# torognes/vsearch

Measured on AMD Instinct MI355X. Metric: GCUPS (useful DP cells/s of the search16 global-alignment path: DP + traceback + CIGAR), higher is better.
Workload: dtype int16

## Files before the change

profiles/tb_stats.py:

```python
import argparse
import ctypes as C
import json
import os
import sys

import numpy as np
import torch

sys.path.insert(0, os.path.dirname(os.path.dirname(os.path.abspath(__file__))))
from vsearch_amd import Aligner, SequenceSet, _lib, workload

ap = argparse.ArgumentParser()
ap.add_argument("--queries", type=int, default=100_000)
ap.add_argument("--qlen", type=int, default=250)
ap.add_argument("--db", type=int, default=1_000_000)
ap.add_argument("--dlen", type=int, default=1000)
a = ap.parse_args()
dev = torch.device("cuda", 0)
db_ascii, db_off, db_len, fam = workload.make_family_db(a.db, a.dlen, seed=17, device=dev)
q_ascii, q_off, q_len, src = workload.make_queries(db_ascii, db_off, db_len, a.queries, a.qlen, seed=11, device=dev)
qidx, tidx = workload.family_candidates(src, fam, per_query=8, seed=5)
torch.cuda.synchronize()
lib = _lib.load()
lib.vsx_internal_tb_stats.argtypes = [C.POINTER(C.c_ulonglong), C.c_int]
out = (C.c_ulonglong * 16)()
with Aligner(device=0) as al:
    T = SequenceSet(al, blob=db_ascii.numel(), offsets=db_off, lengths=db_len, device_ptr=db_ascii.data_ptr())
    Q = SequenceSet(al, blob=q_ascii.numel(), offsets=q_off, lengths=q_len, device_ptr=q_ascii.data_ptr())
    plan = al.plan(Q, T, qidx, tidx)
    lib.vsx_internal_tb_stats(out, 1)
    plan.run()
    tm = plan.sync()
    lib.vsx_internal_tb_stats(out, 1)
    info = plan.describe()
    plan.close()
it, busy, distinct, walked, trips, pairs = (int(out[k]) for k in range(6))
print(json.dumps({"shape": [a.qlen, a.dlen], "pairs": pairs, "tasks": info["tasks"], "rows": info["rows_dominant"],
                  "wave_iterations": it, "busy_pair_tiles": busy, "tiles_per_pair": round(busy / max(pairs, 1), 2),
                  "iterations_per_wave": round(it / max(pairs / 64, 1), 2), "lane_utilisation": round(busy / max(it * 64, 1), 3),
                  "distinct_task_tiles": distinct, "pairs_per_distinct_tile": round(busy / max(distinct, 1), 2),
                  "cells_walked": walked, "cells_walked_per_pair_tile": round(walked / max(busy, 1), 2),
                  "traceback_ms_instrumented": round(tm.traceback_ms, 3),
                  "phase_cycles_per_wave_iteration(load1,recompute1,walk1,load2,recompute2,walk2)": [round(int(out[8 + k]) / max(it, 1)) for k in range(6)],
                  "kernel_cycles_per_wave": round(int(out[15]) / max(pairs / 64, 1))}))
```

vsearch_amd/csrc/vsx_device.hip:

```cpp
#include <hip/hip_runtime.h>
#include <type_traits>
#include <cstdlib>
#include <atomic>
#include "vsx_internal.h"

typedef unsigned int u32;
typedef unsigned int u32x4 __attribute__((ext_vector_type(4)));
typedef unsigned int u32x3 __attribute__((ext_vector_type(3)));
typedef short s2 __attribute__((ext_vector_type(2)));
typedef unsigned short us2 __attribute__((ext_vector_type(2)));

#define DEV __device__ __forceinline__
struct __attribute__((aligned(4))) Pair2 { unsigned int x, y; };

#define SIGN2 0x80008000u

DEV s2 S2(u32 x) { return __builtin_bit_cast(s2, x); }
DEV us2 U2(u32 x) { return __builtin_bit_cast(us2, x); }
DEV u32 UI(s2 x) { return __builtin_bit_cast(u32, x); }
DEV u32 UI(us2 x) { return __builtin_bit_cast(u32, x); }

DEV u32 sadd(u32 a, u32 b) { return UI(__builtin_elementwise_add_sat(S2(a), S2(b))); }
DEV u32 ssub(u32 a, u32 b) { return UI(__builtin_elementwise_sub_sat(S2(a), S2(b))); }
DEV u32 pmax(u32 a, u32 b) { return UI(__builtin_elementwise_max(S2(a), S2(b))); }
// ... 1041 lines not shown
              u32 cv = vin((u32) (uint16_t) P.hleft[ii < 0 ? 0 : ii]);
              if (TOPPAD && L == 0 && xs < pad) cv = vin((u32) (uint16_t) (((xs == pad - 1) ? 0 : -P.top_open) + (xs - pad - 1) * tl));
              tbL[64 + tid] = cv;
            }
        }
      else if (L == 0)
        {
#pragma unroll
          for (int cc = 0; cc < 17; ++cc)
            {
              int c = c0 - 1 + cc;
              if (c > jj) c = jj;
              const u32 corner = (u32) (uint16_t) (((TOPPAD && pad > 0) ? -P.top_open : 0) - (pad + 2) * tl);
              tbL[(cc + 1) * 64 + tid] = (c < 0) ? vin(corner) : vin((u32) (uint16_t) (P.htop[c] - pad * tl));
            }
        }
      else
        {
          const int Lp = L - 1;
          const int sp = Lp >> 4, lp = Lp & 15;
          stage_top(rowck + (size_t) VSX_CK_SLOT(CK8, g, lp) * (CK8 ? 3 : 4), VSX_ROWCK_PAIR_DW(CK8), (long) ((size_t) sp * steps) + (long) (c0 - 1 + lp),
                    (long) (rowsteps >> 1) - 1);
          if (c0 == 0) tbL[64 + tid] = vin((u32) (uint16_t) P.hleft[i0 - 1]);
        }
      stage_symbols(c0);

      u32 hp[RT], ee[RT], qa[RT];
      const u32 qrq_i = pen_pk(P.qrq_i_pk);
      const u32 rq_i = pen_pk(P.rq_i_pk);
      const bool lastrow_here = lastpos && (!MID || hh == 1);
      const u32 qrq_last = lastrow_here ? pen_pk(P.qrq_r_pk) : qrq_i;
      const u32 rq_last = lastrow_here ? pen_pk(P.rq_r_pk) : rq_i;
      if (m == 0)
        {
#pragma unroll
          for (int x = 0; x < RT; ++x)
            {
              int ii = i0 + r0h + x; if (ii > Q - 1) ii = Q - 1;
              if (ii < 0) ii = 0;
              const u32 hl = vin((u32) (uint16_t) P.hleft[ii]);
              hp[x] = hl;
              ee[x] = A::sub(hl, (ii < Q - 1) ? qrq_i : pen_pk(P.qrq_r_pk));
            }
          if (TOPPAD && L == 0 && pad > 0)
            {
#pragma unroll
              for (int x = 0; x < RT; ++x)
                if (r0h + x < pad)
                  {
                    const int xs = r0h + x;
                    const int sh = (xs - pad - 1) * tl;
                    hp[x] = vin((u32) (uint16_t) (((xs == pad - 1) ? 0 : -P.top_open) + sh));
                    ee[x] = A::sub(vin((u32) (uint16_t) (-P.top_open - P.top_step + sh)), qrq_i);
                  }
            }
        }
      else
        {
          if (CK8)
            {
              constexpr int NBQ = MID ? VSX_COLCK_NBH(RT) : VSX_COLCK_NB(R, true);
              Quad fq[NBQ];
              if (MID)
                {
                  const u32 * cb = colck + ((size_t) s * nblk + (size_t) (m - 1)) * COL_DW + VSX_COLCK_CDW(VSX_COLCK_NB(R, true), VSX_CK_SLOT(true, g, l), 0)
                                   + (size_t) (hh * NBQ) * (4 * VSX_COLCK_CG);
#pragma unroll
                  for (int b = 0; b < NBQ; ++b) fq[b] = *reinterpret_cast<const Quad *>(cb + (size_t) b * (4 * VSX_COLCK_CG));
                }
              else
                {
                  const u32 * cb = colck + ((size_t) s * nblk + (size_t) (m - 1)) * COL_DW + VSX_COLCK_CDW(VSX_COLCK_NB(R, true), VSX_CK_SLOT(true, g, l), 0);
#pragma unroll
                  for (int b = 0; b < NBQ; ++b) fq[b] = *reinterpret_cast<const Quad *>(cb + (size_t) b * (4 * VSX_COLCK_CG));
                }
              auto flat = [&](int z) -> u32 {
                const Quad & qd = fq[z >> 2];
                return (z & 3) == 0 ? qd.x : (z & 3) == 1 ? qd.y : (z & 3) == 2 ? qd.z : qd.w;
              };
#pragma unroll
              for (int x = 0; x < RT; ++x)
                {
                  const u32 h = half_lo(flat(x), hi) & 0xffffu;
                  const u32 dd = flat(RT + (x >> 1)) >> (8 * ((x & 1) * 2 + (hi ? 1 : 0)));
                  hp[x] = h;
                  ee[x] = h - (u32) (int) (int8_t) (dd & 0xffu);
                }
            }
          else if (R % 2 == 0)
            {
              const u32 * cb = colck + ((size_t) s * nblk + (size_t) (m - 1)) * COL_DW + VSX_COLCK_DW(R, g * 16 + l, 0);
              constexpr int NBQ = (2 * R) / 4 ? (2 * R) / 4 : 1;
              Quad fq[NBQ];
#pragma unroll
              for (int b = 0; b < NBQ; ++b) fq[b] = *reinterpret_cast<const Quad *>(cb + (size_t) b * (4 * VSX_COLCK_G));
              auto flat = [&](int z) -> u32 {
                const Quad & qd = fq[z >> 2];
                return (z & 3) == 0 ? qd.x : (z & 3) == 1 ? qd.y : (z & 3) == 2 ? qd.z : qd.w;
              };
#pragma unroll
              for (int x = 0; x < R; ++x) { hp[x] = inck(half_lo(flat(x), hi)); ee[x] = inck(half_lo(flat(R + x), hi)); }
            }
          else
            {
#pragma unroll
              for (int x = 0; x < R; ++x)
                {
                  hp[x] = inck(half_lo(colck_at(s, m - 1, g * 16 + l, x), hi));
                  ee[x] = inck(half_lo(colck_at(s, m - 1, g * 16 + l, R + x), hi));
                }
            }
        }
      {
        u32 w[(RT + 3) / 4];
#pragma unroll
        for (int e = 0; e < (RT + 3) / 4; ++e) w[e] = *reinterpret_cast<const u32_unaligned *>(q + i0 + r0h + 4 * e);
#pragma unroll
        for (int x = 0; x < RT; ++x)
          qa[x] = (w[x >> 2] >> (8 * (x & 3))) & 15u;
        if (TOPPAD && L == 0)
          {
#pragma unroll
            for (int x = 0; x < RT; ++x)
              if (r0h + x < pad) qa[x] = 16u;
          }
      }
      u32 diag = tbL[64 + tid] & 0xffffu;

      const bool tile_int = CK8 && RT > 1 && RT <= 16 && !__any(busy && (c0 + cmax >= D - 1));
      const bool top_is_border = (L == 0) && (hh == 0);
      for (int cc = 0; cc <= cmax; ++cc)
        {
          const int c = c0 + cc;
          const u32 qrt = (c < D - 1) ? qrt_i16 : qrt_r16;
          const u32 rt = (c < D - 1) ? rt_i16 : rt_r16;
          const u32 tbv = tbL[(cc + 2) * 64 + tid];
          const u32 topH = tbv & 0xffffu;
          u32 F = top_is_border ? A::sub(topH, qrt) : (tbv >> 16);
          const u32 b16 = (((u32) symL[(cc >> 1) * 64 + tid] >> (4 * (cc & 1))) & 15u) * 32u;
          u32 Hd = diag;
          u32 acc = 0;
          auto row = [&](int x, auto int_tag) __attribute__((always_inline)) {
            constexpr bool INT = decltype(int_tag)::value;
            const u32 V = A::score((int16_t) Ssh[b16 + qa[x]]);
            const u32 h0 = A::add(Hd, V);
            const u32 dU = A::dif(h0, F);
            const u32 h1 = A::max(h0, F);
            const u32 dL = A::dif(h1, ee[x]);
            const u32 h2 = A::max(h1, ee[x]);
            Hd = hp[x];
            hp[x] = h2;
            const bool plain = INT && x < RT - 1;
            const u32 qrq = (x == RT - 1) ? qrq_last : qrq_i;
            const u32 rq = (x == RT - 1) ? rq_last : rq_i;
            const u32 hf = A::sub(h2, qrt);
            const u32 f = INT ? F : A::sub(F, rt);
            const u32 dEU = A::dif(hf, f);
            F = A::max(f, hf);
            const u32 he = plain ? hf : A::sub(h2, qrq);
            const u32 e = plain ? ee[x] : A::sub(ee[x], rq);
            const u32 dEL = A::dif(he, e);
            ee[x] = A::max(e, he);
            acc = A::fun(A::fun(A::fun(A::fun(acc, dU), dL), dEU), dEL);
          };
          if (one_row)
            {
              row(0, std::false_type {});
              bitsL[(cc * ND) * 64 + tid] = (uint16_t) A::one_row_word(acc);
            }
          else
            {
#pragma unroll
              for (int x4 = 0; x4 < RT; x4 += 4)
                if (x4 <= rmax)
                  {
                    if (tile_int)
                      {
#pragma unroll
                        for (int y = 0; y < 4; ++y)
                          if (x4 + y < RT) row(x4 + y, std::true_type {});
                      }
                    else
                      {
#pragma unroll
                        for (int y = 0; y < 4; ++y)
                          if (x4 + y < RT) row(x4 + y, std::false_type {});
                      }
                    bitsL[(cc * ND + (x4 >> 2)) * 64 + tid] = (uint16_t) acc;
                  }
            }
          diag = topH;
        }

      if (busy)
        {
          while (r >= r0h && j >= c0 && (!TOPPAD || i >= 0))
            {
              const int cw = j - c0;
              const int rv = r - r0h;
              const u32 w = bitsL[(cw * ND + (rv >> 2)) * 64 + tid];
              int rid = RT - 4 * (rv >> 2);
              if (rid > 4) rid = 4;
              const u32 bts = A::nibble(w, rid, rv & 3);
              ++al;
              if (op == 1 && (bts & A::EXT_LEFT)) { --j; push(1); }
              else if (op == 2 && (bts & A::EXT_UP)) { --i; --r; push(2); }
              else if (bts & A::LEFT) { if (op != 1) ++ga; --j; push(1); }
              else if (bts & A::UP) { if (op != 2) ++ga; --i; --r; push(2); }
              else { --i; --r; --j; push(0); }
#if VSX_TB_STATS
              atomicAdd(&vsx_tb_stats_dev[3], 1ull);
#endif
            }
          if (r < 0 && L > 0) { --L; r = (L == 0 ? rtop0 : R) - 1; }
        }
    }
#if VSX_TB_STATS
  if (valid) atomicAdd(&vsx_tb_stats_dev[5], 1ull);
#endif
  if (!valid) return;

  VsxPairOut o;
  o.pad = 0; o.nruns = 0; o.run_off = 0;
  if (so.overflow)
    {
      o.score = 32767; o.aligned = 0; o.matches = 0; o.mismatches = 0; o.gaps = 0;
      out[pair_ids[k]] = o;
      rank_note(FL, pair_ids[k], 0u, 32767, 0.0);
      return;
    }
  if (i >= 0) { al += (u32) (i + 1); if (op != 2) ++ga; push_n(2, (u32) (i + 1)); }
  if (j >= 0) { al += (u32) (j + 1); if (op != 1) ++ga; push_n(1, (u32) (j + 1)); }
  if (op >= 0) my[nruns++] = (runlen << 2) | (u32) op;

  u32 ma = 0, mi = 0;
  {
    int qi = Q - 1, tj = D - 1;
    for (u32 x = 0; x < nruns; ++x)
      {
        const u32 w = my[x];
        const int len = (int) (w >> 2);
        const u32 o2 = w & 3u;
        if (o2 == 0)
          {
            for (int b = 0; b < len; b += 8)
              {
                const int rem = (len - b < 8) ? len - b : 8;
                const unsigned long long aw = *reinterpret_cast<const u64_unaligned *>(q + (qi - b - 7));
                const unsigned long long cw = *reinterpret_cast<const u64_unaligned *>(d + (tj - b - 7));
                const unsigned long long ones = 0x0101010101010101ull;
                const unsigned long long x = aw & cw;
                unsigned long long t = (x | (x >> 1) | (x >> 2) | (x >> 3)) & ones;
                if (P.n_mismatch)
                  {
                    const unsigned long long a15 = aw & (aw >> 1) & (aw >> 2) & (aw >> 3);
                    const unsigned long long c15 = cw & (cw >> 1) & (cw >> 2) & (cw >> 3);
                    t &= ~(a15 | c15);
                  }
                t &= ~0ull << (8 * (8 - rem));
                const u32 m8 = (u32) __builtin_popcountll(t);
                ma += m8;
                mi += (u32) rem - m8;
              }
            qi -= len; tj -= len;
          }
        else if (o2 == 1) tj -= len;
        else qi -= len;
      }
  }

  u32 verdict = 0;
  double idv = 0.0;
  if (FL.enabled && nruns > 0) verdict = accept_verdict(FL, Q, D, (int) al, (int) ma, (int) mi, (int) ga, my[nruns - 1], my[0], &idv);
  if (verdict == 3u) nruns = 0;
  rank_note(FL, pair_ids[k], verdict, (int) so.score, idv);

  const unsigned long long base = atomicAdd(cursor, (unsigned long long) nruns);
  if (base + nruns <= runs_capacity)
    for (u32 x = 0; x < nruns; ++x) runs[base + x] = my[x];

  o.score = so.score;
  o.aligned = (uint16_t) al; o.matches = (uint16_t) ma; o.mismatches = (uint16_t) mi; o.gaps = (uint16_t) ga;
  o.pad = (uint16_t) verdict;
  o.nruns = nruns;
  o.run_off = base;
  out[pair_ids[k]] = o;
}


DEV u32 pk_add(u32 a, u32 b) { return UI((us2) (U2(a) + U2(b))); }
DEV u32 pk_sub(u32 a, u32 b) { return psubw(a, b); }
#ifdef VSX_TB2_WAVES_N
#define VSX_TB2_WAVES(R_, MID_) VSX_TB2_WAVES_N
#endif
#ifndef VSX_TB2_WAVES
#define VSX_TB2_WAVES(R_, MID_) 3
#endif
#ifndef VSX_TB_LDSSTAGE
#define VSX_TB_LDSSTAGE 1
#endif
#ifndef VSX_TB_LDSSTAGE_FOR
#define VSX_TB_LDSSTAGE_FOR(R_) ((R_) == 14 || (R_) == 16 || (R_) >= 26)
#endif
template <int R, bool MID>
__global__ void __launch_bounds__(64) __attribute__((amdgpu_waves_per_eu(VSX_TB2_WAVES(R, MID), 8)))
vsx_traceback_tilt_kernel(const VsxDevParams P, const VsxFilterDev FL, const VsxTask * __restrict__ tasks,
                          const u32 * __restrict__ pair_slot, const u32 * __restrict__ pair_ids, u32 npairs,
                          const uint8_t * __restrict__ qc, const uint8_t * __restrict__ tc,
                          const u32 * __restrict__ ck, const VsxSlotOut * __restrict__ slot,
                          u32 * __restrict__ slab, const uint64_t * __restrict__ slab_off,
                          u32 * __restrict__ runs, uint64_t runs_capacity, unsigned long long * cursor,
                          VsxPairOut * __restrict__ out)
{
  static_assert(R >= 4 && (!MID || R % 2 == 0), "R = 1 keeps the first kernel");
  constexpr int RT = MID ? R / 2 : R;
  constexpr int HR = (RT + 1) / 2;
  constexpr int NG = (HR + 3) / 4;
  constexpr int XL = RT - 1 - HR;
  constexpr int NBQ = MID ? VSX_COLCK_NBH(RT) : VSX_COLCK_NB(R, true);
  __shared__ uint8_t Ssh[512];
  __shared__ u32 Ssh4[16];
  constexpr int BITS_DW = 17 * NG * 64, SYM_DW = 10 * 64 / 4;
  __shared__ __attribute__((aligned(16))) u32 arenaL[BITS_DW + SYM_DW + 19 * 64];
  u32 * const bitsL = arenaL;
  uint8_t * const symL = reinterpret_cast<uint8_t *>(arenaL + BITS_DW);
  u32 * const tbL = arenaL + BITS_DW + SYM_DW;
  constexpr bool LSTAGE = (VSX_TB_LDSSTAGE != 0) && VSX_TB_LDSSTAGE_FOR(R) && (BITS_DW + SYM_DW >= 9 * 64 * 4);
  const int tid = (int) threadIdx.x;
  for (int x = tid; x < 512; x += 64)
    Ssh[x] = (uint8_t) (((x & 31) < 16) ? P.matrix[(x >> 5) * 16 + (x & 15)] : (int16_t) (-P.top_step + 2 * P.tilt));
  if (tid < 16)
    {
      const int16_t * mr = P.matrix + tid * 16;
      Ssh4[tid] = (u32) (uint8_t) mr[1] | ((u32) (uint8_t) mr[2] << 8) | ((u32) (uint8_t) mr[4] << 16) | ((u32) (uint8_t) mr[8] << 24);
    }
  __syncthreads();

  const u32 k = blockIdx.x * 64 + (u32) threadIdx.x;
  const bool valid = k < npairs;
  const u32 ts = pair_slot[valid ? k : 0];
  const u32 task = ts >> 3, sl = ts & 7;
  const VsxTask & T = tasks[task];
  const VsxSlotOut so = slot[ts];
  const bool live = valid && !so.overflow;

  const int Q = (int) T.qlen;
  const int D = (int) T.tlen[sl];
  const u32 steps32 = T.steps;
  const unsigned long long dir_off = T.dir_off;
  constexpr size_t COL_DW = (size_t) 64 * 4 * VSX_COLCK_NB(R, true);
  const int g = (int) (sl >> 1) + (int) T.group0;
  const bool hi = (sl & 1) != 0;
  const u32 half_sel = hi ? 0x07060302u : 0x05040100u;
  const u32 bias = P.max3 ? 0x3E00u : 0x8000u;
  const u32 bias_pk = bias * 0x10001u;
  const int tl = P.tilt;
  auto pk16 = [](int v) -> u32 { const u32 x = (u32) v & 0xffffu; return x | (x << 16); };
  auto pk2 = [](int lo, int hi_) -> u32 { return ((u32) lo & 0xffffu) | ((u32) hi_ << 16); };
  const int qrt_i = P.qrt_i, qrt_r = P.qrt_r, rt_i = P.rt_i, rt_r = P.rt_r;
  const int qrq_i = (int) (int16_t) (P.qrq_i_pk & 0xffffu), rq_i = (int) (int16_t) (P.rq_i_pk & 0xffffu);
  const int qrq_r = (int) (int16_t) (P.qrq_r_pk & 0xffffu), rq_r = (int) (int16_t) (P.rq_r_pk & 0xffffu);
  const uint8_t * __restrict__ q = qc + T.qoff;
  const uint8_t * __restrict__ d = tc + T.toff[sl];
  u32 * __restrict__ my = slab + slab_off[valid ? k : 0];

  int i = live ? Q - 1 : -1, j = live ? D - 1 : -1;
  int L = (Q + R - 1) / R - 1;
  int r = R - 1;
  int op = -1;
  u32 runlen = 0, nruns = 0;
  u32 al = 0, ga = 0;
  auto push_n = [&](int newop, u32 n) {
    if (newop == op) { runlen += n; return; }
    if (op >= 0) my[nruns++] = (runlen << 2) | (u32) op;
    op = newop;
    runlen = n;
  };
  auto push = [&](int newop) { push_n(newop, 1u); };

  if (live)
    {
      const int lv = (so.leave == 0xFFFFu) ? -1 : (int) so.leave;
      if (lv < D - 1)
        {
          const u32 n = (u32) (D - 1 - lv);
          al += n; ++ga;
          push_n(1, n);
          j = lv;
        }
    }

  const u32 mA[4] = {0x01010101u, 0x02020202u, 0x04040404u, 0x08080808u};
  const u32 mB[4] = {0x10101010u, 0x20202020u, 0x40404040u, 0x80808080u};

#if VSX_TB_STATS
  const unsigned long long t_kernel0 = __builtin_readcyclecounter();
  unsigned n_iter = 0;
  unsigned long long tphase[6] = {0, 0, 0, 0, 0, 0};
#endif
  for (;;)
    {
      const bool busy = (i >= 0) && (j >= 0);
      if (!__any(busy)) break;
#if VSX_TB_STATS
      ++n_iter;
#endif

      u32 Qb = (u32) Q, stb = steps32;
      unsigned long long dob = dir_off;
      asm volatile("" : "+v"(Qb), "+v"(stb), "+v"(dob));
      const int total_lanes = ((int) Qb + R - 1) / R;
      const int rcnt0 = (int) Qb - (total_lanes - 1) * R;
      const int pad = R - rcnt0;
      const int nstrips = (total_lanes + 15) >> 4;
      const size_t steps = stb;
      const size_t nblk = (steps + 15) >> 4;
      const size_t rowsteps = ((size_t) nstrips * steps + 1) & ~(size_t) 1;
      const size_t rowck_dw = (rowsteps >> 1) * VSX_ROWCK_PAIR_DW(true);
      const u32 * __restrict__ rowck = ck + dob;
      const u32 * __restrict__ colck = rowck + rowck_dw;
      const u32 * __restrict__ midck = colck + (size_t) nstrips * nblk * COL_DW;
      const int s = L >> 4, l = L & 15;
      const int jj = busy ? j : 0;
      const int m = (jj + l) >> 4;
      const int c0 = (16 * m - l) > 0 ? 16 * m - l : 0;
      const int c0b = (m >= 1 && 16 * (m - 1) - l > 0) ? 16 * (m - 1) - l : 0;
      const int i0 = (L == 0) ? -pad : rcnt0 + (L - 1) * R;
      const bool lastpos = (L == total_lanes - 1);
      const int hh = (MID && busy && r >= RT) ? 1 : 0;
      const int r0h = hh * RT;
      const bool lastrow_here = lastpos && (!MID || hh == 1);
      const bool top_is_border = (L == 0) && (hh == 0);
#if VSX_TB_STATS & 1
      {
        const unsigned key = busy ? (((unsigned) task & 0x3FFu) << 22) | ((unsigned) L << 12) | ((unsigned) m << 1) | (unsigned) hh : 0xFFFFFFFFu;
        bool leader = busy;
        for (int o = 1; o < 8; ++o)
          {
            const unsigned other = (unsigned) __shfl((int) key, (tid & ~7) | ((tid - o) & 7), 64);
            if ((tid & 7) >= o && other == key) leader = false;
          }
        const unsigned long long nb = __popcll(__ballot(busy)), nl = __popcll(__ballot(leader));
        if (tid == 0) { atomicAdd(&vsx_tb_stats_dev[1], nb); atomicAdd(&vsx_tb_stats_dev[2], nl); }
      }
#endif

      struct TileIn { Trio v3[LSTAGE ? 1 : 9]; int par; Quad fq[NBQ]; u32 sw[5]; };
      auto load_tile = [&](TileIn & in, const int cst, const int mleft) __attribute__((always_inline)) {
        in.par = 0;
        if (!top_is_border)
          {
            const u32 * base;
            long gstart;
            if (MID && hh == 1)
              {
                base = midck + (size_t) VSX_CK_SLOT(true, g, l) * 3;
                gstart = (long) ((size_t) s * steps) + (long) (cst - 1 + l);
              }
            else
              {
                const int Lp = L - 1, sp = Lp >> 4, lp = Lp & 15;
                base = rowck + (size_t) VSX_CK_SLOT(true, g, lp) * 3;
                gstart = (long) ((size_t) sp * steps) + (long) (cst - 1 + lp);
              }
            const long p0 = gstart >> 1;
            in.par = (int) (gstart - 2 * p0);
            const u32 * bp = base + p0 * (long) VSX_ROWCK_PAIR_DW(true);
            if (LSTAGE)
              {
#pragma unroll
                for (int e = 0; e < 9; ++e)
                  __builtin_amdgcn_global_load_lds((const __attribute__((address_space(1))) void *) (bp + e * VSX_ROWCK_PAIR_DW(true)),
                                                   (__attribute__((address_space(3))) void *) (arenaL + e * 256), 12, 0, 0);
              }
            else
              {
#pragma unroll
            for (int e = 0; e < 9; ++e) in.v3[LSTAGE ? 0 : e] = *reinterpret_cast<const Trio *>(bp + e * VSX_ROWCK_PAIR_DW(true));
              }
          }
        const u32 * cb = colck + ((size_t) s * nblk + (size_t) (mleft > 0 ? mleft : 0)) * COL_DW + VSX_COLCK_CDW(VSX_COLCK_NB(R, true), VSX_CK_SLOT(true, g, l), 0)
                         + (MID ? (size_t) (hh * NBQ) * (4 * VSX_COLCK_CG) : 0);
#pragma unroll
        for (int b = 0; b < NBQ; ++b) in.fq[b] = *reinterpret_cast<const Quad *>(cb + (size_t) b * (4 * VSX_COLCK_CG));
#pragma unroll
        for (int e = 0; e < 5; ++e) in.sw[e] = *reinterpret_cast<const u32_unaligned *>(d + cst + 4 * e);
      };

      u32 qcd[HR], qsel[HR];
      bool plain_acgt = true;
      {
        u32 w[(RT + 3) / 4];
#pragma unroll
        for (int e = 0; e < (RT + 3) / 4; ++e) w[e] = *reinterpret_cast<const u32_unaligned *>(q + i0 + r0h + 4 * e);
        auto code_of = [&](int x) -> u32 {
          const int xx = x < RT ? x : RT - 1;
          u32 c = (w[xx >> 2] >> (8 * (xx & 3))) & 15u;
          if (L == 0 && r0h + xx < pad) c = 16u;
          return c;
        };
#pragma unroll
        for (int x = 0; x < HR; ++x)
          {
            const u32 a = code_of(x), b = code_of(x + HR);
            qcd[x] = a | (b << 16);
            const u32 ia = (a >> 1) - (a >> 3), ib = (b >> 1) - (b >> 3);
            qsel[x] = ia | 0x0C000C00u | ((4u + ib) << 16);
            plain_acgt = plain_acgt && (a == 1 || a == 2 || a == 4 || a == 8) && (b == 1 || b == 2 || b == 4 || b == 8);
          }
      }
      const bool fastV = !__any(busy && !plain_acgt);

      const u32 qrq_pk_i = pk16(qrq_i), rq_pk_i = pk16(rq_i);
      const u32 qrq_pk_x = pk2(qrq_i, lastrow_here ? qrq_r : qrq_i), rq_pk_x = pk2(rq_i, lastrow_here ? rq_r : rq_i);

      auto recompute = [&](const TileIn & in, const bool border_left, const int cst, const int rmax_raw, const int cmax, const bool tile_int)
                       __attribute__((always_inline)) {
        if (top_is_border)
          {
            const u32 corner = (u32) (uint16_t) (((pad > 0) ? -P.top_open : 0) - (pad + 2) * tl);
#pragma unroll
            for (int e = 0; e < 17; ++e)
              {
                int c = cst - 1 + e;
                if (c > jj) c = jj;
                tbL[e * 64 + tid] = (c < 0) ? (corner & 0xffffu) : (u32) (uint16_t) (P.htop[c] - pad * tl);
              }
          }
        else
          {
            u32 * dst = tbL + tid - in.par * 64;
            if (LSTAGE) asm volatile("s_waitcnt vmcnt(0)" ::: "memory");
#pragma unroll
            for (int e = 0; e < 9; ++e)
              {
                Trio raw;
                if (LSTAGE) raw = *reinterpret_cast<const Trio *>(arenaL + e * 256 + tid * 4);
                else raw = in.v3[LSTAGE ? 0 : e];
                const u32 h0 = (half_lo(raw.x, hi) - bias) & 0xffffu, h1 = (half_lo(raw.y, hi) - bias) & 0xffffu;
                const u32 dd = hi ? (raw.z >> 8) : raw.z;
                const int d0 = (int) (int8_t) (dd & 0xffu), d1 = (int) (int8_t) ((dd >> 16) & 0xffu);
                if (e > 0 || in.par == 0) dst[(2 * e) * 64] = h0 | ((h0 - (u32) d0) << 16);
                dst[(2 * e + 1) * 64] = h1 | ((h1 - (u32) d1) << 16);
              }
            if (cst == 0)
              {
                u32 cv;
                if (MID && hh == 1)
                  {
                    const int xs = RT - 1;
                    int ii = i0 + xs; if (ii > Q - 1) ii = Q - 1;
                    cv = (u32) (uint16_t) P.hleft[ii < 0 ? 0 : ii];
                    if (L == 0 && xs < pad) cv = (u32) (uint16_t) (((xs == pad - 1) ? 0 : -P.top_open) + (xs - pad - 1) * tl);
                  }
                else cv = (u32) (uint16_t) P.hleft[i0 - 1];
                tbL[tid] = cv;
              }
          }
#pragma unroll
        for (int c2 = 0; c2 < 10; ++c2)
          {
            const u32 lo = (in.sw[c2 >> 1] >> (16 * (c2 & 1))) & 15u, hi4 = (in.sw[c2 >> 1] >> (16 * (c2 & 1) + 8)) & 15u;
            symL[c2 * 64 + tid] = (uint8_t) (lo | (hi4 << 4));
          }
        u32 hp[HR], ee[HR];
        if (border_left)
          {
#pragma unroll
            for (int x = 0; x < HR; ++x)
              {
                u32 hv[2], ev[2];
#pragma unroll
                for (int hf_ = 0; hf_ < 2; ++hf_)
                  {
                    const int xs = r0h + x + hf_ * HR;
                    int ii = i0 + xs; if (ii > Q - 1) ii = Q - 1;
                    if (ii < 0) ii = 0;
                    asm volatile("" : "+v"(ii));
                    int hl = P.hleft[ii];
                    int e0 = hl - ((ii < Q - 1) ? qrq_i : qrq_r);
                    if (L == 0 && xs < pad)
                      {
                        const int sh = (xs - pad - 1) * tl;
                        hl = ((xs == pad - 1) ? 0 : -P.top_open) + sh;
                        e0 = -P.top_open - P.top_step + sh - qrq_i;
                      }
                    hv[hf_] = (u32) hl & 0xffffu; ev[hf_] = (u32) e0 & 0xffffu;
                  }
                hp[x] = hv[0] | (hv[1] << 16);
                ee[x] = ev[0] | (ev[1] << 16);
              }
          }
        else
          {
            auto flat = [&](int z) -> u32 {
              const Quad & qd = in.fq[z >> 2];
              return (z & 3) == 0 ? qd.x : (z & 3) == 1 ? qd.y : (z & 3) == 2 ? qd.z : qd.w;
            };
#pragma unroll
            for (int x = 0; x < HR; ++x)
              {
                const int xa = x, xb = (x + HR < RT) ? x + HR : RT - 1;
                const u32 h = pk_sub(__builtin_amdgcn_perm(flat(xb), flat(xa), half_sel), bias_pk);
                const int da = (int) (int8_t) ((flat(RT + (xa >> 1)) >> (8 * ((xa & 1) * 2 + (hi ? 1 : 0)))) & 0xffu);
                const int db = (int) (int8_t) ((flat(RT + (xb >> 1)) >> (8 * ((xb & 1) * 2 + (hi ? 1 : 0)))) & 0xffu);
                hp[x] = h;
                ee[x] = pk_sub(h, ((u32) da & 0xffffu) | ((u32) db << 16));
              }
          }
        const int xmax = rmax_raw >= HR ? HR - 1 : rmax_raw;
        u32 tb_prev = tbL[tid];
        u32 Hd_end = 0, F_end = 0;
        u32 cr_prev = 0, qrt_prev = 0, rt_prev = 0;
        auto sym_at = [&](int it) -> u32 { return ((u32) symL[(it >> 1) * 64 + tid] >> (4 * (it & 1))) & 15u; };
        const bool FASTV_any = fastV;
        u32 tbv_n = tbL[64 + tid];
        u32 cr_n = FASTV_any ? Ssh4[sym_at(0)] : sym_at(0) * 32u;
        u32 sy_n = sym_at(1);
        auto column = [&](const int it, auto int_tag, auto fast_tag, auto first_tag) __attribute__((always_inline)) {
          constexpr bool INT = decltype(int_tag)::value;
          constexpr bool FASTV = decltype(fast_tag)::value;
          constexpr bool FIRST = decltype(first_tag)::value;
          const int c = cst + it;
          const u32 tbv = tbv_n;
          const u32 cr = cr_n;
          cr_n = FASTV ? Ssh4[sy_n] : sy_n * 32u;
          tbv_n = tbL[(it + 2) * 64 + tid];
          sy_n = sym_at(it + 2);
          u32 qrt_pk = 0, rt_pk = 0;
          if (!INT)
            {
              const u32 ql = (u32) ((c < D - 1) ? qrt_i : qrt_r) & 0xffffu, rl = (u32) ((c < D - 1) ? rt_i : rt_r) & 0xffffu;
              qrt_pk = ql | (qrt_prev << 16); rt_pk = rl | (rt_prev << 16);
              qrt_prev = ql; rt_prev = rl;
            }
          else qrt_pk = pk16(qrt_i);
          u32 Hd = __builtin_amdgcn_perm(Hd_end, tb_prev, 0x05040100u);
          u32 F = __builtin_amdgcn_perm(F_end, tbv, 0x05040302u);
          if (top_is_border)
            F = __builtin_amdgcn_perm(F_end, ((tbv & 0xffffu) - (INT ? (u32) qrt_i : (qrt_pk & 0xffffu))), 0x05040100u);
#pragma unroll
          for (int g4 = 0; g4 < NG; ++g4)
            if (4 * g4 <= xmax)
              {
                u32 acc = 0;
#pragma unroll
                for (int x = 4 * g4; x < 4 * g4 + 4; ++x)
                  if (x < HR)
                    {
                      u32 V;
                      if (FASTV) V = __builtin_amdgcn_perm(cr_prev, cr, qsel[x]);
                      else
                        {
                          u32 qc2 = qcd[x];
                          asm volatile("" : "+v"(qc2));
                          V = (u32) Ssh[cr + (qc2 & 0xffffu)] | ((u32) Ssh[cr_prev + (qc2 >> 16)] << 16);
                        }
                      const u32 h0 = pk_add(Hd, V);
                      const u32 dU = ssub(h0, F);
                      const u32 h1 = pmax(h0, F);
                      const u32 dL = ssub(h1, ee[x]);
                      const u32 h2 = pmax(h1, ee[x]);
                      Hd = hp[x];
                      hp[x] = FIRST ? bfi(0x0000FFFFu, h2, hp[x]) : h2;
                      const u32 hf = pk_sub(h2, qrt_pk);
                      const u32 f = INT ? F : pk_sub(F, rt_pk);
                      const u32 dEU = ssub(hf, f);
                      F = pmax(f, hf);
                      const bool plain = INT && x != XL;
                      const u32 he = plain ? hf : pk_sub(h2, x == XL ? qrq_pk_x : qrq_pk_i);
                      const u32 e = plain ? ee[x] : pk_sub(ee[x], x == XL ? rq_pk_x : rq_pk_i);
                      const u32 dEL = ssub(he, e);
                      const u32 en = pmax(e, he);
                      ee[x] = FIRST ? bfi(0x0000FFFFu, en, ee[x]) : en;
                      acc = a_bfi(mA[x & 3], __builtin_amdgcn_perm(dL, dU, 0x0B0A0908u), acc);
                      acc = a_bfi(mB[x & 3], __builtin_amdgcn_perm(dEL, dEU, 0x0B0A0908u), acc);
                    }
                bitsL[(it * NG + g4) * 64 + tid] = acc;
              }
          Hd_end = Hd;
          F_end = F;
          tb_prev = tbv;
          cr_prev = cr;
        };
        auto sweep = [&](auto int_tag, auto fast_tag) __attribute__((always_inline)) {
          column(0, int_tag, fast_tag, std::true_type {});
          for (int it = 1; it <= cmax + 1; ++it) column(it, int_tag, fast_tag, std::false_type {});
        };
        if (tile_int) { if (fastV) sweep(std::true_type {}, std::true_type {}); else sweep(std::true_type {}, std::false_type {}); }
        else          { if (fastV) sweep(std::false_type {}, std::true_type {}); else sweep(std::false_type {}, std::false_type {}); }
      };
      auto walk = [&](const int cst) __attribute__((always_inline)) {
        while (r >= r0h && j >= cst && i >= 0)
          {
            const int cw = j - cst;
            const int rv = r - r0h;
            const bool up_half = rv >= HR;
            const int rx = up_half ? rv - HR : rv;
            const u32 w = bitsL[((cw + (up_half ? 1 : 0)) * NG + (rx >> 2)) * 64 + tid] >> ((rx & 3) + (up_half ? 8 : 0));
            ++al;
            const u32 inI = (op == 1) ? 1u : 0u, inD = (op == 2) ? 1u : 0u;
            const u32 c1 = inI & (w >> 20);
            const u32 c2 = (c1 ^ 1u) & inD & (w >> 4);
            const u32 c12 = c1 | c2;
            const u32 c3 = (c12 ^ 1u) & (w >> 16);
            const u32 c4 = ((c12 | c3) ^ 1u) & w;
            const u32 isI = (c1 | c3) & 1u, isD = (c2 | c4) & 1u;
            const int newop = (int) (isI + 2u * isD);
            ga += ((c3 & (inI ^ 1u)) | (c4 & (inD ^ 1u))) & 1u;
            j -= (int) (isD ^ 1u);
            const int di = (int) (isI ^ 1u);
            i -= di; r -= di;
            if (newop != op)
              {
                if (op >= 0) my[nruns++] = (runlen << 2) | (u32) op;
                op = newop;
                runlen = 0;
              }
            ++runlen;
#if VSX_TB_STATS & 1
            atomicAdd(&vsx_tb_stats_dev[3], 1ull);
#endif
          }
      };

#if VSX_TB_STATS & 2
#define TBMARK(k_) do { __builtin_amdgcn_s_waitcnt(0); const unsigned long long now_ = __builtin_readcyclecounter(); tphase[k_] += now_ - tmark; tmark = now_; } while (0)
      unsigned long long tmark = __builtin_readcyclecounter();
#else
#define TBMARK(k_) do { } while (0)
#endif
#pragma unroll 1
      for (int tno = 0; tno < 2; ++tno)
        {
          const bool need = (tno == 0) ? busy : (busy && (m >= 1) && (r >= r0h) && (i >= 0) && (j >= 0) && (j < c0));
          if (tno == 1 && !__any(need)) break;
          const int cst = tno ? c0b : c0;
          TileIn in;
          load_tile(in, cst, tno ? m - 2 : m - 1);
          TBMARK(3 * tno);
          const int rmax_raw = __builtin_amdgcn_readfirstlane(wave_max_i32(need ? r - r0h : 0));
          const int cmax = __builtin_amdgcn_readfirstlane(wave_max_i32(need ? j - cst : 0));
          const bool tile_int = tno ? true : !__any(busy && (c0 + cmax >= D - 1));
          recompute(in, tno ? (m <= 1) : (m == 0), cst, rmax_raw, cmax, tile_int);
          TBMARK(3 * tno + 1);
          if (need) walk(cst);
          TBMARK(3 * tno + 2);
        }
      if (busy && r < 0 && L > 0) { --L; r = R - 1; }
    }
#if VSX_TB_STATS
  if (valid) atomicAdd(&vsx_tb_stats_dev[5], 1ull);
  if (tid == 0)
    {
      atomicAdd(&vsx_tb_stats_dev[15], __builtin_readcyclecounter() - t_kernel0); atomicAdd(&vsx_tb_stats_dev[0], (unsigned long long) n_iter);
      for (int k2 = 0; k2 < 6; ++k2) atomicAdd(&vsx_tb_stats_dev[8 + k2], tphase[k2]);
    }
#endif
  if (!valid) return;

  VsxPairOut o;
  o.pad = 0; o.nruns = 0; o.run_off = 0;
  if (so.overflow)
    {
      o.score = 32767; o.aligned = 0; o.matches = 0; o.mismatches = 0; o.gaps = 0;
      out[pair_ids[k]] = o;
      rank_note(FL, pair_ids[k], 0u, 32767, 0.0);
      return;
    }
  if (i >= 0) { al += (u32) (i + 1); if (op != 2) ++ga; push_n(2, (u32) (i + 1)); }
  if (j >= 0) { al += (u32) (j + 1); if (op != 1) ++ga; push_n(1, (u32) (j + 1)); }
  if (op >= 0) my[nruns++] = (runlen << 2) | (u32) op;

  u32 ma = 0, mi = 0;
  {
    int qi = Q - 1, tj = D - 1;
    for (u32 x = 0; x < nruns; ++x)
      {
        const u32 w = my[x];
        const int len = (int) (w >> 2);
        const u32 o2 = w & 3u;
        if (o2 == 0)
          {
            for (int b = 0; b < len; b += 8)
              {
                const int rem = (len - b < 8) ? len - b : 8;
                const unsigned long long aw = *reinterpret_cast<const u64_unaligned *>(q + (qi - b - 7));
                const unsigned long long cw = *reinterpret_cast<const u64_unaligned *>(d + (tj - b - 7));
                const unsigned long long ones = 0x0101010101010101ull;
                const unsigned long long x2 = aw & cw;
                unsigned long long t = (x2 | (x2 >> 1) | (x2 >> 2) | (x2 >> 3)) & ones;
                if (P.n_mismatch)
                  {
                    const unsigned long long a15 = aw & (aw >> 1) & (aw >> 2) & (aw >> 3);
                    const unsigned long long c15 = cw & (cw >> 1) & (cw >> 2) & (cw >> 3);
                    t &= ~(a15 | c15);
                  }
                t &= ~0ull << (8 * (8 - rem));
                const u32 m8 = (u32) __builtin_popcountll(t);
                ma += m8;
                mi += (u32) rem - m8;
              }
            qi -= len; tj -= len;
          }
        else if (o2 == 1) tj -= len;
        else qi -= len;
      }
  }

  u32 verdict = 0;
  double idv = 0.0;
  if (FL.enabled && nruns > 0) verdict = accept_verdict(FL, Q, D, (int) al, (int) ma, (int) mi, (int) ga, my[nruns - 1], my[0], &idv);
  if (verdict == 3u) nruns = 0;
  rank_note(FL, pair_ids[k], verdict, (int) so.score, idv);

  const unsigned long long base = atomicAdd(cursor, (unsigned long long) nruns);
  if (base + nruns <= runs_capacity)
    for (u32 x = 0; x < nruns; ++x) runs[base + x] = my[x];

  o.score = so.score;
  o.aligned = (uint16_t) al; o.matches = (uint16_t) ma; o.mismatches = (uint16_t) mi; o.gaps = (uint16_t) ga;
  o.pad = (uint16_t) verdict;
  o.nruns = nruns;
  o.run_off = base;
  out[pair_ids[k]] = o;
}

DEV u32 map4(u32 ch)
{
  const u32 c = ch | 0x20u;
  if (((ch | 0x20u) < 'a') || ((ch | 0x20u) > 'z') || ((ch & 0xC0u) != 0x40u)) return 0;
  switch (c)
    {
    case 'a': return 1;  case 'b': return 14; case 'c': return 2;  case 'd': return 13;
    case 'g': return 4;  case 'h': return 11; case 'k': return 12; case 'm': return 3;
    case 'n': return 15; case 'r': return 5;  case 's': return 6;  case 't': return 8;
    case 'u': return 8;  case 'v': return 7;  case 'w': return 9;  case 'y': return 10;
    default: return 0;
    }
}

__global__ void __launch_bounds__(256)
vsx_encode_kernel(const uint8_t * __restrict__ ascii, uint8_t * __restrict__ codes, uint64_t nbytes)
{
  __shared__ uint8_t lut[256];
  lut[threadIdx.x] = (uint8_t) map4(threadIdx.x);
  __syncthreads();
  const uint64_t nvec = nbytes >> 4;
  const uint64_t stride = (uint64_t) gridDim.x * blockDim.x;
  for (uint64_t v = (uint64_t) blockIdx.x * blockDim.x + threadIdx.x; v < nvec; v += stride)
    {
      const uint4 in = reinterpret_cast<const uint4 *>(ascii)[v];
      u32 w[4] = {in.x, in.y, in.z, in.w};
      u32 o[4];
#pragma unroll
      for (int x = 0; x < 4; ++x)
        o[x] = (u32) lut[w[x] & 0xff] | ((u32) lut[(w[x] >> 8) & 0xff] << 8) |
               ((u32) lut[(w[x] >> 16) & 0xff] << 16) | ((u32) lut[w[x] >> 24] << 24);
      reinterpret_cast<uint4 *>(codes)[v] = make_uint4(o[0], o[1], o[2], o[3]);
    }
  if (blockIdx.x == 0 && threadIdx.x < (nbytes & 15))
    {
      const uint64_t p = (nvec << 4) + threadIdx.x;
      codes[p] = lut[ascii[p]];
    }
}

__global__ void __launch_bounds__(256)
vsx_purity_kernel(const uint8_t * __restrict__ codes, const uint64_t * __restrict__ off,
                  const uint32_t * __restrict__ len, uint64_t nseq, uint8_t * __restrict__ impure)
{
  const uint64_t s = (uint64_t) blockIdx.x * 4 + (threadIdx.x >> 6);
  if (s >= nseq) return;
  const int lane = threadIdx.x & 63;
  const uint8_t * p = codes + off[s];
  const uint32_t n = len[s];
  int bad = 0;
  for (uint32_t x = lane; x < n; x += 64)
    {
      const u32 c = p[x];
      bad |= !((c != 0) && ((c & (c - 1)) == 0));
    }
  const unsigned long long any = __ballot(bad);
  if (lane == 0) impure[s] = any ? 1 : 0;
}

__global__ void __launch_bounds__(256)
vsx_max3_selftest_kernel(u32 * bad)
{
  const u32 x = blockIdx.x * 256u + threadIdx.x;
  if (x > 0x7BFFu) return;
  const u32 edge[8] = {0u, 1u, 0x03FFu, 0x0400u, 0x3C00u, 0x3E00u, 0x7BFEu, 0x7BFFu};
  u32 wrong = 0;
  for (u32 k = 0; k < 64; ++k)
    {
      const u32 h = (x * 2654435761u) ^ (k * 0x9E3779B9u);
      const u32 y = (k < 8) ? edge[k] : (h >> 7) % 0x7C00u;
      const u32 z = (k < 16) ? edge[(k + 3) & 7] : (h >> 17) % 0x7C00u;
      const u32 a = x | (y << 16), b = y | (z << 16), c = z | (x << 16);
      const u32 got = pk_max3_bits(a, b, c);
      const u32 m = x > y ? (x > z ? x : z) : (y > z ? y : z);
      if (got != (m | (m << 16))) ++wrong;
      const u32 pa = h ^ (x << 13), pb = (h * 0x85EBCA6Bu) ^ k;
      const u32 pg = __builtin_amdgcn_perm(pa, pb, 0x0B0A0908u);
      const u32 pe = ((pb >> 15) & 1u) * 0xFFu | (((pb >> 31) & 1u) * 0xFFu) << 8 | (((pa >> 15) & 1u) * 0xFFu) << 16 | (((pa >> 31) & 1u) * 0xFFu) << 24;
      if (pg != pe) atomicAdd(bad + 1, 1u);
    }
  if (wrong) atomicAdd(bad, wrong);
}
static std::atomic<int> g_tb_v1_dev[65];
extern "C" void vsx_internal_set_tb_v2(int device, int on) { g_tb_v1_dev[device < 0 || device > 64 ? 64 : device].store(on ? 0 : 1); }
extern "C" hipError_t vsx_launch_max3_selftest(u32 * d_bad, hipStream_t st)
{
  hipLaunchKernelGGL(vsx_max3_selftest_kernel, dim3((0x7C00 + 255) / 256), dim3(256), 0, st, d_bad);
  return hipGetLastError();
}

static const int kRows[] = {1, 4, 8, 10, 12, 14, 16, 18, 20, 22, 24, 26, 28, 32};

extern "C" const int * vsx_supported_rows(int * count)
{
  *count = (int) (sizeof(kRows) / sizeof(kRows[0]));
  return kRows;
}

extern "C" hipError_t vsx_launch_encode(const uint8_t * d_ascii, uint8_t * d_codes, uint64_t nbytes, hipStream_t st)
{
  if (nbytes == 0) return hipSuccess;
  uint64_t blocks = ((nbytes >> 4) + 255) / 256;
  if (blocks < 1) blocks = 1;
  if (blocks > 256 * 8) blocks = 256 * 8;
  hipLaunchKernelGGL(vsx_encode_kernel, dim3((unsigned) blocks), dim3(256), 0, st, d_ascii, d_codes, nbytes);
  return hipGetLastError();
}

extern "C" hipError_t vsx_launch_purity(const uint8_t * d_codes, const uint64_t * d_off, const uint32_t * d_len,
                                        uint64_t nseq, uint8_t * d_impure, hipStream_t st)
{
  if (nseq == 0) return hipSuccess;
  hipLaunchKernelGGL(vsx_purity_kernel, dim3((unsigned) ((nseq + 3) / 4)), dim3(256), 0, st,
                     d_codes, d_off, d_len, nseq, d_impure);
  return hipGetLastError();
}

#define VSX_FWD_GO(GRID_, ...) hipLaunchKernelGGL((vsx_forward_kernel<__VA_ARGS__>), dim3(GRID_), dim3(64), 0, st, P, d_tasks, q, t, dir, strip, slot, ntasks)
#define VSX_FWD_GO4(GRID_, ...) hipLaunchKernelGGL((vsx_forward_kernel<__VA_ARGS__>), dim3(GRID_), dim3(256), 0, st, P, d_tasks, q, t, dir, strip, slot, ntasks)
template <int R>
static hipError_t launch_fwd2(int track, int nq, int one, const VsxDevParams & P, const VsxTask * d_tasks, uint32_t ntasks,
                              const uint8_t * q, const uint8_t * t, uint32_t * dir, uint2 * strip,
                              VsxSlotOut * slot, hipStream_t st)
{
  if (nq == 8)
    {
      if (!(P.tilt != 0 && !track) || (ntasks & 3u)) return hipErrorInvalidValue;
      if constexpr (R >= 4)
        {
          if (!one) return hipErrorInvalidValue;
          if (P.max3) VSX_FWD_GO4(ntasks / 4, R, false, true, true, 1, true, true); else VSX_FWD_GO4(ntasks / 4, R, false, true, false, 1, true, true);
          return hipGetLastError();
        }
      else return hipErrorInvalidValue;
    }
  if (nq == 16)
    {
      if (!(P.tilt != 0 && P.max3 && !track && one)) return hipErrorInvalidValue;
      if constexpr (VSX_SPLIT_ROWS(R))
        {
          VSX_FWD_GO(ntasks, R, false, true, true, 1, false, true, true);
          return hipGetLastError();
        }
      else return hipErrorInvalidValue;
    }
  if (nq != 1)
    {
      if (!(P.tilt != 0 && !track && (nq == 2 || nq == 4))) return hipErrorInvalidValue;
      if constexpr (R >= 4)
        {
          const uint32_t grid = (ntasks + (uint32_t) nq - 1) / (uint32_t) nq;
          if (nq == 2) { if (P.max3) VSX_FWD_GO(grid, R, false, true, true, 2); else VSX_FWD_GO(grid, R, false, true, false, 2); }
          else         { if (P.max3) VSX_FWD_GO(grid, R, false, true, true, 4); else VSX_FWD_GO(grid, R, false, true, false, 4); }
          return hipGetLastError();
        }
      else return hipErrorInvalidValue;
    }
  if (P.tilt != 0)
    {
      if (track) return hipErrorInvalidValue;
      if constexpr (R >= 4)
        {
          if (one)
            {
              if (P.max3) VSX_FWD_GO(ntasks, R, false, true, true, 1, false, true);
              else VSX_FWD_GO(ntasks, R, false, true, false, 1, false, true);
              return hipGetLastError();
            }
        }
      if (P.max3) VSX_FWD_GO(ntasks, R, false, true, true);
      else VSX_FWD_GO(ntasks, R, false, true);
    }
  else if (track) VSX_FWD_GO(ntasks, R, true);
  else VSX_FWD_GO(ntasks, R, false);
  return hipGetLastError();
}
#undef VSX_FWD_GO
#undef VSX_FWD_GO4

extern "C" hipError_t vsx_launch_forward(int rows, int track, int nq, int one, VsxDevParams P, const VsxTask * d_tasks, uint32_t ntasks,
                                         const uint8_t * q, const uint8_t * t, uint32_t * dir, uint2 * strip,
                                         VsxSlotOut * slot, hipStream_t st)
{
  if (ntasks == 0) return hipSuccess;
#define FWDR(RR) case RR: return launch_fwd2<RR>(track, nq, one, P, d_tasks, ntasks, q, t, dir, strip, slot, st)
  switch (rows)
    {
    FWDR(1); FWDR(4); FWDR(8); FWDR(10); FWDR(12); FWDR(14); FWDR(16); FWDR(18); FWDR(20); FWDR(22); FWDR(24); FWDR(26); FWDR(28); FWDR(32);
    default: return hipErrorInvalidValue;
    }
#undef FWDR
}

template <int R, bool MID>
static hipError_t launch_tbtilt(const VsxDevParams & P, const VsxFilterDev & F, const VsxTask * d_tasks, const uint32_t * d_pair_slot,
                                const uint32_t * d_pair_ids, uint32_t npairs, const uint8_t * q, const uint8_t * t,
                                const uint32_t * ck, const VsxSlotOut * slot, uint32_t * slab, const uint64_t * slab_off,
                                uint32_t * runs, uint64_t cap, unsigned long long * cursor, VsxPairOut * out, hipStream_t st)
{
  if constexpr (R >= 4)
    hipLaunchKernelGGL((vsx_traceback_tilt_kernel<R, MID>), dim3((npairs + 63) / 64), dim3(64), 0, st,
                       P, F, d_tasks, d_pair_slot, d_pair_ids, npairs, q, t, ck, slot, slab, slab_off, runs, cap, cursor, out);
  return hipGetLastError();
}

template <int R, bool FAST, bool CK8 = false, bool MID = false>
static hipError_t launch_tbck(const VsxDevParams & P, const VsxFilterDev & F, const VsxTask * d_tasks, const uint32_t * d_pair_slot,
                              const uint32_t * d_pair_ids, uint32_t npairs, const uint8_t * q, const uint8_t * t,
                              const uint32_t * ck, const VsxSlotOut * slot, uint32_t * slab, const uint64_t * slab_off,
                              uint32_t * runs, uint64_t cap, unsigned long long * cursor, VsxPairOut * out, hipStream_t st)
{
  hipLaunchKernelGGL((vsx_traceback_ck_kernel<R, FAST, CK8, MID>), dim3((npairs + 127) / 128), dim3(128), 0, st,
                     P, F, d_tasks, d_pair_slot, d_pair_ids, npairs, q, t, ck, slot, slab, slab_off, runs, cap, cursor, out);
  return hipGetLastError();
}

extern "C" hipError_t vsx_launch_traceback_ck(int rows, int fast16, VsxDevParams P, VsxFilterDev F, const VsxTask * d_tasks, const uint32_t * d_pair_slot,
                                              const uint32_t * d_pair_ids, uint32_t npairs,
                                              const uint8_t * q, const uint8_t * t,
                                              const uint32_t * ck, const VsxSlotOut * slot,
                                              uint32_t * slab, const uint64_t * slab_off,
                                              uint32_t * runs, uint64_t runs_capacity, unsigned long long * cursor,
                                              VsxPairOut * out, hipStream_t st)
{
  if (npairs == 0) return hipSuccess;
  int dev_now = 0;
  if (hipGetDevice(&dev_now) != hipSuccess) { (void) hipGetLastError(); dev_now = 64; }
  const bool v2 = g_tb_v1_dev[dev_now < 0 || dev_now > 64 ? 64 : dev_now].load(std::memory_order_relaxed) == 0;
#define TBCK(RR) case RR: return (fast16 && P.tilt != 0 && v2 && RR >= 4) ? launch_tbtilt<RR, VSX_MID(RR, true)>(P, F, d_tasks, d_pair_slot, d_pair_ids, npairs, q, t, ck, slot, slab, slab_off, runs, runs_capacity, cursor, out, st) \
                                 : (fast16 && P.tilt != 0) ? launch_tbck<RR, true, true, VSX_MID(RR, true)>(P, F, d_tasks, d_pair_slot, d_pair_ids, npairs, q, t, ck, slot, slab, slab_off, runs, runs_capacity, cursor, out, st) \
                                 : fast16 ? launch_tbck<RR, true>(P, F, d_tasks, d_pair_slot, d_pair_ids, npairs, q, t, ck, slot, slab, slab_off, runs, runs_capacity, cursor, out, st) \
// ... 24 lines not shown
```

Measured before the change: 9424.

## Batch traceback walk over diagonal match runs using prefetched bit words

The traceback walk now loads up to four direction-bit words along the diagonal in one step and, when the current step is a diagonal move, advances over consecutive diagonal cells until a stop bit appears. Each walk loop trip can therefore cover several cells, cutting the serial per-cell LDS load and branch latency in the divergent walk. The cost is extra LDS loads per trip, more complex index math, and a sched barrier. Stats instrumentation also gains a trip counter and batches the per-cell atomic.

```diff
diff --git a/profiles/tb_stats.py b/profiles/tb_stats.py
--- a/profiles/tb_stats.py
+++ b/profiles/tb_stats.py
@@ -40,6 +40,7 @@
                   "iterations_per_wave": round(it / max(pairs / 64, 1), 2), "lane_utilisation": round(busy / max(it * 64, 1), 3),
                   "distinct_task_tiles": distinct, "pairs_per_distinct_tile": round(busy / max(distinct, 1), 2),
                   "cells_walked": walked, "cells_walked_per_pair_tile": round(walked / max(busy, 1), 2),
+                  "walk_trips": trips, "walk_trips_per_position": round(trips / max(it, 1), 2),
                   "traceback_ms_instrumented": round(tm.traceback_ms, 3),
                   "phase_cycles_per_wave_iteration(load1,recompute1,walk1,load2,recompute2,walk2)": [round(int(out[8 + k]) / max(it, 1)) for k in range(6)],
                   "kernel_cycles_per_wave": round(int(out[15]) / max(pairs / 64, 1))}))
diff --git a/vsearch_amd/csrc/vsx_device.hip b/vsearch_amd/csrc/vsx_device.hip
--- a/vsearch_amd/csrc/vsx_device.hip
+++ b/vsearch_amd/csrc/vsx_device.hip
@@ -1367,6 +1367,10 @@
 #ifndef VSX_TB_LDSSTAGE_FOR
 #define VSX_TB_LDSSTAGE_FOR(R_) ((R_) == 14 || (R_) == 16 || (R_) >= 26)
 #endif
+#ifndef VSX_TB_WALK_BATCH
+#define VSX_TB_WALK_BATCH 4
+#endif
+static_assert(VSX_TB_WALK_BATCH >= 1 && VSX_TB_WALK_BATCH <= 16, "a batch stays inside one 16-column tile");
 template <int R, bool MID>
 __global__ void __launch_bounds__(64) __attribute__((amdgpu_waves_per_eu(VSX_TB2_WAVES(R, MID), 8)))
 vsx_traceback_tilt_kernel(const VsxDevParams P, const VsxFilterDev FL, const VsxTask * __restrict__ tasks,
@@ -1382,6 +1386,7 @@
   constexpr int HR = (RT + 1) / 2;
   constexpr int NG = (HR + 3) / 4;
   constexpr int XL = RT - 1 - HR;
+  constexpr int WB = VSX_TB_WALK_BATCH;
   constexpr int NBQ = MID ? VSX_COLCK_NBH(RT) : VSX_COLCK_NB(R, true);
   __shared__ uint8_t Ssh[512];
   __shared__ u32 Ssh4[16];
@@ -1460,7 +1465,7 @@
 
 #if VSX_TB_STATS
   const unsigned long long t_kernel0 = __builtin_readcyclecounter();
-  unsigned n_iter = 0;
+  unsigned n_iter = 0, n_trips = 0, n_cells = 0;
   unsigned long long tphase[6] = {0, 0, 0, 0, 0, 0};
 #endif
   for (;;)
@@ -1756,13 +1761,34 @@
         else          { if (fastV) sweep(std::false_type {}, std::true_type {}); else sweep(std::false_type {}, std::false_type {}); }
       };
       auto walk = [&](const int cst) __attribute__((always_inline)) {
+#if VSX_TB_STATS
+        unsigned ntrip = 0;
+#endif
         while (r >= r0h && j >= cst && i >= 0)
           {
             const int cw = j - cst;
             const int rv = r - r0h;
             const bool up_half = rv >= HR;
             const int rx = up_half ? rv - HR : rv;
-            const u32 w = bitsL[((cw + (up_half ? 1 : 0)) * NG + (rx >> 2)) * 64 + tid] >> ((rx & 3) + (up_half ? 8 : 0));
+            u32 wk[WB], shk[WB];
+            shk[0] = (u32) ((rx & 3) + (up_half ? 8 : 0));
+            wk[0] = bitsL[((cw + (up_half ? 1 : 0)) * NG + (rx >> 2)) * 64 + tid];
+            const int kmax = min(min(rv, cw), min(i, WB - 1));
+            static_assert(NG <= 2, "4 NG is a single bit of the virtual row");
+#pragma unroll
+            for (int k2 = 1; k2 < WB; ++k2)
+              {
+                const int kk = min(k2, kmax);
+                const int rvk = rv - kk;
+                const int v = (4 * NG != HR && rvk >= HR) ? rvk + (4 * NG - HR) : rvk;
+                shk[k2] = (u32) ((v & 3) | ((v & (4 * NG)) << (NG == 2 ? 0 : 1)));
+                wk[k2] = bitsL[((cw - kk) * NG + (v >> 2)) * 64 + tid];
+              }
+            if (WB > 1) __builtin_amdgcn_sched_barrier(0);
+            const u32 w = wk[0] >> shk[0];
+#if VSX_TB_STATS
+            ++ntrip;
+#endif
             ++al;
             const u32 inI = (op == 1) ? 1u : 0u, inD = (op == 2) ? 1u : 0u;
             const u32 c1 = inI & (w >> 20);
@@ -1783,10 +1809,24 @@
                 runlen = 0;
               }
             ++runlen;
+            u32 nd = 0;
+            if (WB > 1)
+              {
+                u32 stop = 0;
+#pragma unroll
+                for (int k2 = 1; k2 < WB; ++k2) stop |= ((wk[k2] >> shk[k2]) & 0x00010001u) << (k2 - 1);
+                stop |= (stop >> 16) | (1u << kmax);
+                nd = (newop == 0) ? (u32) __builtin_ctz(stop) : 0u;
+                al += nd; runlen += nd;
+                i -= (int) nd; r -= (int) nd; j -= (int) nd;
+              }
 #if VSX_TB_STATS & 1
-            atomicAdd(&vsx_tb_stats_dev[3], 1ull);
+            n_cells += 1u + nd;
 #endif
           }
+#if VSX_TB_STATS
+        return ntrip;
+#endif
       };
 
 #if VSX_TB_STATS & 2
@@ -1809,16 +1849,22 @@
           const bool tile_int = tno ? true : !__any(busy && (c0 + cmax >= D - 1));
           recompute(in, tno ? (m <= 1) : (m == 0), cst, rmax_raw, cmax, tile_int);
           TBMARK(3 * tno + 1);
+#if VSX_TB_STATS
+          n_trips += (unsigned) wave_max_i32(need ? (int) walk(cst) : 0);
+#else
           if (need) walk(cst);
+#endif
           TBMARK(3 * tno + 2);
         }
       if (busy && r < 0 && L > 0) { --L; r = R - 1; }
     }
 #if VSX_TB_STATS
   if (valid) atomicAdd(&vsx_tb_stats_dev[5], 1ull);
+  if (n_cells) atomicAdd(&vsx_tb_stats_dev[3], (unsigned long long) n_cells);
   if (tid == 0)
     {
       atomicAdd(&vsx_tb_stats_dev[15], __builtin_readcyclecounter() - t_kernel0); atomicAdd(&vsx_tb_stats_dev[0], (unsigned long long) n_iter);
+      atomicAdd(&vsx_tb_stats_dev[4], (unsigned long long) n_trips);
       for (int k2 = 0; k2 < 6; ++k2) atomicAdd(&vsx_tb_stats_dev[8 + k2], tphase[k2]);
     }
 #endif
```

Result: faster. 9522, median of 6 (+1.0%).
